# facebookresearch/pytorchvideo

Measured on AMD Instinct MI355X. Metric: clips/sec forward, higher is better.
Workload: dtype bf16; 1 GPU; x3d_m: create_x3d(input_clip_length=16,input_crop_size=224) [B,3,16,224,224]; per_gpu_batch=32, global_batch=32, parallelism=dp1 (batch-sharded, logits all_gather), head_collective=none (one rank: the logits stay where they are), hip_graph=True, streams=2

## Files before the change

### pytorchvideo_amd/accelerator/mi355x/emit.py

```python
import ctypes as C

import torch
import torch.nn as nn

from ... import _lib as L
from . import tuning
from .session import Ptr, pad8


class Unsupported(Exception):
    pass


def _cls_name(m):
    return getattr(m, "_orig_cls", type(m)).__name__


def _is_a(m, types):
    return issubclass(getattr(m, "_orig_cls", type(m)), types)


def act_code(act):
    if act is None or isinstance(act, nn.Identity):
        return L.ACT_NONE
# ... 484 lines not shown
        if getattr(se, "is_3d", True) is not True:
            raise Unsupported("2-D squeeze-excitation")
        _se_parts(se, x.C)
        y, psum, nblk = emit_dwconv(sess, conv_b, x, bn, L.ACT_NONE, want_psum=True, label="conv_b.dw+se")
        gate = emit_se_gate(sess, se, psum, nblk, x.B, x.C, y.voxels)
        sess.release(psum)
        return y, gate, act
    y = emit_conv(sess, conv_b, x, bn, act, label="conv_b")
    return y, None, L.ACT_NONE


def _conv_bc_desc(sess, bb, a, residual, out):
    conv_b, conv_c = bb.conv_b, bb.conv_c
    if not isinstance(conv_b, nn.Conv3d) or not isinstance(conv_c, nn.Conv3d) or sess.itemsize != 2 or a.f32:
        return None
    if conv_b.padding_mode != "zeros" or isinstance(conv_b.padding, str) or conv_c.padding_mode != "zeros" \
            or isinstance(conv_c.padding, str):
        return None
    bn, se = _split_norm_b(bb.norm_b)
    if se is not None or conv_b.groups != 1 or tuple(conv_b.dilation) != (1, 1, 1) or conv_b.in_channels != a.C:
        return None
    if conv_c.kernel_size != (1, 1, 1) or tuple(conv_c.stride) != (1, 1, 1) or _triple(conv_c.padding) != (0, 0, 0) \
            or conv_c.groups != 1 or conv_c.in_channels != conv_b.out_channels:
        return None
    if a.ld < pad8(a.C) or (residual is not None and residual.f32):
        return None
    kt, kh, kw = conv_b.kernel_size
    st, sh, sw = conv_b.stride
    pt, ph, pw = _triple(conv_b.padding)
    To, Ho, Wo = _conv_out(a.T, kt, st, pt), _conv_out(a.H, kh, sh, ph), _conv_out(a.W, kw, sw, pw)
    if min(To, Ho, Wo) <= 0 or kt * kh * kw == 1:
        return None
    cout2 = conv_c.out_channels
    if out is not None:
        if (out.B, out.T, out.H, out.W, out.C) != (a.B, To, Ho, Wo, cout2) or out.f32:
            return None
        ldy, y_bs = out.ld, out.bs
    else:
        ldy, y_bs = pad8(cout2), To * Ho * Wo * pad8(cout2)
    if residual is not None and ((residual.B, residual.T, residual.H, residual.W, residual.C) != (a.B, To, Ho, Wo, cout2)
                                 or residual.ld != ldy or residual.bs != y_bs):
        return None
    return dict(x_bs=a.bs, y_bs=y_bs, r_bs=y_bs if residual is not None else 0, ldx=a.ld, ldy=ldy,
                ldr=ldy if residual is not None else 0, B=a.B, Ti=a.T, Hi=a.H, Wi=a.W, cin=pad8(a.C), To=To, Ho=Ho, Wo=Wo,
                cout=conv_b.out_channels, kt=kt, kh=kh, kw=kw, st=st, sh=sh, sw=sw, pt=pt, ph=ph, pw=pw,
                dtype=sess.pv_dtype, pw2_cout=cout2)


def can_fuse_conv_bc(sess, bb, a, residual, out, shortcut):
    if not tuning.get("fuse_bc") or shortcut is not None:
        return False
    g = _conv_bc_desc(sess, bb, a, residual, out)
    if g is None:
        return False
    d = L.Conv3dDesc()
    for k, v in g.items():
        setattr(d, k, v)
    return L.lib().pv_conv3d_pw2_supported(C.byref(d)) == 1


def emit_fused_conv_bc(sess, bb, a, residual, final_act, out=None):
    g = _conv_bc_desc(sess, bb, a, residual, out)
    conv_b, conv_c = bb.conv_b, bb.conv_c
    bn, _ = _split_norm_b(bb.norm_b)
    cb, cc, cin_p = conv_b.out_channels, conv_c.out_channels, pad8(a.C)
    taps = g["kt"] * g["kh"] * g["kw"]
    y = out if out is not None else sess.alloc_act(a.B, g["To"], g["Ho"], g["Wo"], cc)
    wb = torch.zeros(cb, taps, cin_p, dtype=torch.float32)
    wb[:, :, : a.C] = conv_b.weight.detach().float().cpu().permute(0, 2, 3, 4, 1).reshape(cb, taps, a.C)
    wc = torch.zeros(cc, pad8(cb), dtype=torch.float32)
    wc[:, :cb] = conv_c.weight.detach().float().cpu().reshape(cc, cb)
    scale_b, shift_b = fold_norm(bn, cb, conv_b.bias)
    scale_c, shift_c = fold_norm(bb.norm_c, cc, conv_c.bias)
    aff_b = bn is not None and not isinstance(bn, nn.Identity)
    aff_c = bb.norm_c is not None and not isinstance(bb.norm_c, nn.Identity)
    f = dict(g)
    f.update(x=a.ptr, w=sess.add_weight(wb.to(sess.dtype)), y=y.ptr,
             scale=sess.add_weight(scale_b) if aff_b else None,
             shift=sess.add_weight(shift_b) if (aff_b or conv_b.bias is not None) else None,
             residual=residual.ptr if residual is not None else None,
             act=act_code(bb.act_b), a_act=L.ACT_NONE,
             pw2_w=sess.add_weight(wc.to(sess.dtype)),
             pw2_scale=sess.add_weight(scale_c) if aff_c else None,
             pw2_shift=sess.add_weight(shift_c) if (aff_c or conv_c.bias is not None) else None,
             pw2_act=final_act)
    vox_in, vox_out = a.B * a.voxels, y.B * y.voxels
    alg = sess.itemsize * (vox_in * cin_p + cb * taps * cin_p + cc * pad8(cb) + vox_out * pad8(cc)
                           + (vox_out * pad8(cc) if residual is not None else 0))
    flops = 2 * vox_out * (cb * taps * a.C + cc * cb)
    sess.add_op(L.OP_CONV3D, f, label="conv_bc|%dx%dx%dx%d c%d->%d->%d k%dx%dx%d s%d%d%d+k1x1x1" % (
        a.B, g["To"], g["Ho"], g["Wo"], a.C, cb, cc, g["kt"], g["kh"], g["kw"], g["st"], g["sh"], g["sw"]),
        alg_bytes=alg, flops=flops)
    return y


def emit_bottleneck(sess, bb, x, residual=None, final_act=L.ACT_NONE, out=None, shortcut=None):
    for name in ("conv_a", "conv_b", "conv_c"):
        if getattr(bb, name, None) is None:
            raise Unsupported("bottleneck without %s" % name)
    if can_fuse_bottleneck_ab(sess, bb, x):
        b, gate, deferred = emit_fused_conv_ab_se(sess, bb, x)
    elif can_fuse_pointwise_into_dw(sess, bb.conv_a, bb.conv_b, x):
        b, gate, deferred = emit_conv_b(sess, bb.conv_b, x, bb.norm_b, bb.act_b,
                                        producer=(bb.conv_a, bb.norm_a, act_code(bb.act_a)))
    else:
        a = emit_conv(sess, bb.conv_a, x, bb.norm_a, act_code(bb.act_a), label="conv_a")
        if can_fuse_conv_bc(sess, bb, a, residual, out, shortcut):
            c = emit_fused_conv_bc(sess, bb, a, residual, final_act, out=out)
            sess.release(a)
            return c
        b, gate, deferred = emit_conv_b(sess, bb.conv_b, a, bb.norm_b, bb.act_b)
        sess.release(a)
    check_conv3d(bb.conv_c)
    if (gate is not None or deferred != L.ACT_NONE) and \
            (bb.conv_c.kernel_size != (1, 1, 1) or bb.conv_c.stride != (1, 1, 1) or _triple(bb.conv_c.padding) != (0, 0, 0)):
        raise Unsupported("SE block whose conv_c is not pointwise")
    c = emit_conv(sess, bb.conv_c, b, bb.norm_c, final_act, residual=residual, a_gate=gate, a_act=deferred,
                  out=out, label="conv_c", shortcut=shortcut)
    sess.release(b)
    if gate is not None:
        sess.release(gate)
    return c


def pack_bottleneck_operands(conv_a, norm_a, conv_b, bn_b, conv_c, norm_c):
    cin, Cc = conv_a.in_channels, conv_a.out_channels
    cout = conv_c.out_channels if conv_c is not None else 16
    Cp, cin_p = (Cc + 31) // 32 * 32, (cin + 31) // 32 * 32

    def frag_image(w, rows_p, cols_p):
        wp = torch.zeros(rows_p, cols_p, dtype=torch.float32)
        wp[:w.shape[0], :w.shape[1]] = w
        return wp.reshape(rows_p // 16, 16, cols_p // 32, 4, 8).permute(0, 2, 3, 1, 4).contiguous().to(torch.bfloat16).reshape(-1)

    wa = frag_image(conv_a.weight.detach().float().cpu().reshape(Cc, cin), Cp, cin_p)
    wc = frag_image(conv_c.weight.detach().float().cpu().reshape(cout, Cc), (cout + 15) // 16 * 16, Cp) if conv_c is not None else None
    wb = torch.zeros(27, Cp, dtype=torch.float32)
    wb[:, :Cc] = conv_b.weight.detach().float().cpu().reshape(Cc, 27).t()

    def padded(v, n):
        o = torch.zeros(n, dtype=torch.float32)
        o[:v.numel()] = v
        return o

    sa, ha = fold_norm(norm_a, Cc, conv_a.bias)
    sb, hb = fold_norm(bn_b, Cc, conv_b.bias)
    out = dict(wa=wa, wb=wb.reshape(-1), sa=padded(sa, Cp), ha=padded(ha, Cp), sb=padded(sb, Cp), hb=padded(hb, Cp))
    if conv_c is not None:
        sc, hc = fold_norm(norm_c, cout, conv_c.bias)
        out.update(wc=wc, sc=sc, hc=hc)
    return out


def _bottleneck_geometry_ok(sess, bb, x, want_se):
    if not tuning.get("fuse_block") or sess.itemsize != 2 or x.f32:
        return None
    ca, cb, cc = getattr(bb, "conv_a", None), getattr(bb, "conv_b", None), getattr(bb, "conv_c", None)
    if not all(isinstance(c, nn.Conv3d) for c in (ca, cb, cc)):
        return None
    try:
        bn_b, se = _split_norm_b(bb.norm_b)
        if (se is not None) != want_se or check_conv3d(ca) or not check_conv3d(cb) or check_conv3d(cc) or group_width(cb) != 1:
            return None
        if se is not None:
            if getattr(se, "is_3d", True) is not True:
                return None
            _se_parts(se, cb.out_channels)
        acts = (act_code(bb.act_a), act_code(bb.act_b))
    except Unsupported:
        return None
    for c in (ca, cc):
        if c.kernel_size != (1, 1, 1) or c.stride != (1, 1, 1) or _triple(c.padding) != (0, 0, 0) or c.groups != 1:
            return None
    if cb.kernel_size != (3, 3, 3) or cb.stride != (1, 1, 1) or _triple(cb.padding) != (1, 1, 1) or _triple(cb.dilation) != (1, 1, 1):
        return None
    if ca.in_channels != x.C or ca.out_channels != cb.in_channels or cb.out_channels != cc.in_channels:
        return None
    if x.bs != x.voxels * x.ld:
        return None
    return acts


def can_fuse_bottleneck(sess, bb, x, residual, final_act=L.ACT_RELU):
    if residual is not x:
        return False
    acts = _bottleneck_geometry_ok(sess, bb, x, want_se=False)
    if acts is None or bb.conv_c.out_channels != x.C:
        return False
    d = L.BottleneckDesc()
    d.B, d.T, d.H, d.W, d.cin, d.C, d.cout = x.B, x.T, x.H, x.W, x.C, bb.conv_a.out_channels, bb.conv_c.out_channels
    d.ldx, d.ldy, d.ldr, d.dtype, d.mode = x.ld, pad8(bb.conv_c.out_channels), x.ld, sess.pv_dtype, L.BLOCK_FULL
    d.act_a, d.act_b, d.act_out = acts[0], acts[1], final_act
    return L.lib().pv_bottleneck_supported(C.byref(d)) == 1


def can_fuse_bottleneck_ab(sess, bb, x):
    acts = _bottleneck_geometry_ok(sess, bb, x, want_se=True)
    if acts is None:
        return False
    d = L.BottleneckDesc()
    d.B, d.T, d.H, d.W, d.cin, d.C, d.cout = x.B, x.T, x.H, x.W, x.C, bb.conv_a.out_channels, bb.conv_c.out_channels
    d.ldx, d.ldy, d.dtype, d.mode, d.act_a = x.ld, pad8(bb.conv_a.out_channels), sess.pv_dtype, L.BLOCK_AB, acts[0]
    return L.lib().pv_bottleneck_supported(C.byref(d)) == 1


def emit_fused_conv_ab_se(sess, bb, x):
    bn_b, se = _split_norm_b(bb.norm_b)
    ops = pack_bottleneck_operands(bb.conv_a, bb.norm_a, bb.conv_b, bn_b, None, None)
    cin, Cc = bb.conv_a.in_channels, bb.conv_a.out_channels
    y = sess.alloc_act(x.B, x.T, x.H, x.W, Cc)
    f = dict(x=x.ptr, y=y.ptr, residual=None, wc=None, sc=None, hc=None, x_bs=x.bs, y_bs=y.bs, r_bs=0, ldx=x.ld, ldy=y.ld, ldr=0,
             B=x.B, T=x.T, H=x.H, W=x.W, cin=cin, C=Cc, cout=bb.conv_c.out_channels,
             act_a=act_code(bb.act_a), act_b=L.ACT_NONE, act_out=L.ACT_NONE, dtype=sess.pv_dtype, mode=L.BLOCK_AB)
    for k in ("wa", "wb", "sa", "ha", "sb", "hb"):
        f[k] = sess.add_weight(ops[k])
    d = L.BottleneckDesc()
    d.H, d.W, d.cin, d.C, d.cout, d.ldx, d.mode, d.dtype = x.H, x.W, cin, Cc, bb.conv_c.out_channels, x.ld, L.BLOCK_AB, sess.pv_dtype
    nblk = L.lib().pv_bottleneck_psum_blocks(C.byref(d))
    if nblk <= 0:
        raise Unsupported("bottleneck geometry")
    psum = sess.alloc_raw(4 * x.B * nblk * pad8(Cc))
    f["psum"] = psum
    vox = x.B * x.T * x.H * x.W
    sess.add_op(L.OP_BOTTLENECK, f, label="conv_ab.fused+se|%dx%dx%dx%d c%d->%d k1x1x1+k3x3x3 psum" % (x.B, x.T, x.H, x.W, cin, Cc),
                alg_bytes=sess.itemsize * vox * (pad8(cin) + pad8(Cc)) + 2 * Cc * cin + 108 * Cc, flops=2 * vox * Cc * (cin + 27))
    gate = emit_se_gate(sess, se, psum, nblk, x.B, Cc, x.T * x.H * x.W)
    sess.release(psum)
    return y, gate, act_code(bb.act_b)


def emit_fused_bottleneck(sess, bb, x, final_act, out=None):
    bn_b, _ = _split_norm_b(bb.norm_b)
    ops = pack_bottleneck_operands(bb.conv_a, bb.norm_a, bb.conv_b, bn_b, bb.conv_c, bb.norm_c)
    cin, Cc, cout = bb.conv_a.in_channels, bb.conv_a.out_channels, bb.conv_c.out_channels
    y = out if out is not None else sess.alloc_act(x.B, x.T, x.H, x.W, cout)
    f = dict(x=x.ptr, y=y.ptr, residual=x.ptr, x_bs=x.bs, y_bs=y.bs, r_bs=x.bs, ldx=x.ld, ldy=y.ld, ldr=x.ld,
             B=x.B, T=x.T, H=x.H, W=x.W, cin=cin, C=Cc, cout=cout,
             act_a=act_code(bb.act_a), act_b=act_code(bb.act_b), act_out=final_act, dtype=sess.pv_dtype, mode=L.BLOCK_FULL, psum=None)
    for k in ("wa", "wb", "wc", "sa", "ha", "sb", "hb", "sc", "hc"):
        f[k] = sess.add_weight(ops[k])
    vox = x.B * x.T * x.H * x.W
    sess.add_op(L.OP_BOTTLENECK, f, label="block.fused|%dx%dx%dx%d c%d->%d->%d k1x1x1+k3x3x3+k1x1x1" % (x.B, x.T, x.H, x.W, cin, Cc, cout),
                alg_bytes=sess.itemsize * vox * (pad8(cin) + pad8(cout)) + 2 * Cc * (cin + cout) + 108 * Cc,
                flops=2 * vox * Cc * (cin + cout + 27))
    return y


def emit_res_block(sess, rb, x, out=None):
    if not is_add_fusion(rb.branch_fusion):
        raise Unsupported("branch_fusion is not a sum")
    if _cls_name(rb.branch2) != "BottleneckBlock":
        raise Unsupported("branch2 is %s" % _cls_name(rb.branch2))
    bb = rb.branch2
    if rb.branch1_conv is not None and isinstance(getattr(bb, "conv_c", None), nn.Conv3d) \
            and can_fold_shortcut(sess, bb.conv_c, rb.branch1_conv, x, bb.conv_c.in_channels):
        return emit_bottleneck(sess, bb, x, residual=None, final_act=act_code(rb.activation), out=out,
                               shortcut=(rb.branch1_conv, rb.branch1_norm, x))
    if rb.branch1_conv is None and can_fuse_bottleneck(sess, bb, x, x, act_code(rb.activation)):
        return emit_fused_bottleneck(sess, bb, x, act_code(rb.activation), out=out)
    if rb.branch1_conv is None:
        shortcut = x
    else:
        shortcut = emit_conv(sess, rb.branch1_conv, x, rb.branch1_norm, L.ACT_NONE, label="shortcut")
    y = emit_bottleneck(sess, rb.branch2, x, residual=shortcut, final_act=act_code(rb.activation), out=out)
    if shortcut is not x:
        sess.release(shortcut)
    return y


def emit_res_stage(sess, stage, x, out=None):
    cur = x
    n = len(stage.res_blocks)
    for i, blk in enumerate(stage.res_blocks):
        if _cls_name(blk) != "ResBlock":
            raise Unsupported("stage element %s" % _cls_name(blk))
        nxt = emit_res_block(sess, blk, cur, out=out if i == n - 1 else None)
        if cur is not x:
            sess.release(cur)
        cur = nxt
    return cur


def can_fuse_temporal_dw(sess, first, second, mid_norm, mid_act, x, act):
    if not tuning.get("fuse_stem") or x.ld != 4 or sess.itemsize != 2:
        return False
    if mid_norm is not None and not isinstance(mid_norm, nn.Identity):
        return False
    if mid_act != L.ACT_NONE or not isinstance(first, nn.Conv3d) or not isinstance(second, nn.Conv3d):
        return False
    try:
        if check_conv3d(first) or not check_conv3d(second):
            return False
    except Unsupported:
        return False
    if group_width(second) != 1:
        return False
    k = second.kernel_size
    if first.bias is not None or first.out_channels != second.in_channels or second.in_channels != second.out_channels:
        return False
    if k[1:] != (1, 1) or second.stride != (1, 1, 1) or _triple(second.padding) != (k[0] // 2, 0, 0) or k[0] % 2 == 0:
        return False
    kt, kh, kw = first.kernel_size
    st, sh, sw = first.stride
    pt, ph, pw = _triple(first.padding)
    d = L.Conv3dDesc()
    d.ldx, d.cin, d.cout, d.dtype, d.act, d.dwt_k = 4, 4, first.out_channels, sess.pv_dtype, act, k[0]
    d.B, d.Ti, d.Hi, d.Wi = x.B, x.T, x.H, x.W
    d.To, d.Ho, d.Wo = _conv_out(x.T, kt, st, pt), _conv_out(x.H, kh, sh, ph), _conv_out(x.W, kw, sw, pw)
    d.kt, d.kh, d.kw, d.st, d.sh, d.sw, d.pt, d.ph, d.pw = kt, kh, kw, st, sh, sw, pt, ph, pw
    return min(d.To, d.Ho, d.Wo) > 0 and L.lib().pv_conv3d_dwt_supported(C.byref(d)) == 1


def emit_stem(sess, stem, x, out=None):
    act = act_code(stem.activation)
    conv = stem.conv
    if _cls_name(conv) == "Conv2plus1d":
        first, second = (conv.conv_xy, conv.conv_t) if conv.conv_xy_first else (conv.conv_t, conv.conv_xy)
        if can_fuse_temporal_dw(sess, first, second, conv.norm, act_code(conv.activation), x, act):
            y = emit_conv(sess, first, x, stem.norm, act, out=out if stem.pool is None else None,
                          label="stem.conv01", dwt=second)
        else:
            mid = emit_conv(sess, first, x, conv.norm, act_code(conv.activation), label="stem.conv0")
            y = emit_conv(sess, second, mid, stem.norm, act, out=out if stem.pool is None else None,
                          label="stem.conv1")
            sess.release(mid)
    else:
        y = emit_conv(sess, conv, x, stem.norm, act, out=out if stem.pool is None else None, label="stem.conv")
    if stem.pool is not None:
        p = emit_pool(sess, stem.pool, y, out=out, label="stem.pool")
        sess.release(y)
        y = p
    return y


def _emit_linear_rows(sess, lin, x, act=L.ACT_NONE, y_f32=False, label="linear"):
    if not isinstance(lin, nn.Linear):
        raise Unsupported("%s is not nn.Linear" % _cls_name(lin))
    if lin.in_features != x.C:
        raise RuntimeError("Linear expects %d features, got %d" % (lin.in_features, x.C))
    conv = nn.Conv3d(lin.in_features, lin.out_features, 1, bias=lin.bias is not None)
    conv.weight.data = lin.weight.detach().reshape(lin.out_features, lin.in_features, 1, 1, 1)
    if lin.bias is not None:
        conv.bias.data = lin.bias.detach()
    return emit_conv(sess, conv, x, None, act, y_f32=y_f32, label=label)


def emit_projected_pool(sess, pp, x):
    a = emit_conv(sess, pp.pre_conv, x, pp.pre_norm, act_code(pp.pre_act), label="head.pre_conv")
    p = emit_pool(sess, pp.pool, a, label="head.pool")
    sess.release(a)
    y = emit_conv(sess, pp.post_conv, p, pp.post_norm, act_code(pp.post_act), label="head.post_conv")
    sess.release(p)
    return y


def emit_res_head(sess, head, x):
    cur = x
    if head.pool is not None:
        if _cls_name(head.pool) == "ProjectedPool":
            cur = emit_projected_pool(sess, head.pool, x)
        else:
            cur = emit_pool(sess, head.pool, x, label="head.pool")
    if head.dropout is not None and not isinstance(head.dropout, nn.Dropout):
        raise Unsupported("head dropout %s" % _cls_name(head.dropout))
    a = head.activation
    if a is not None and not isinstance(a, (nn.Softmax, nn.Sigmoid, nn.ReLU)):
        raise Unsupported("head activation %s" % _cls_name(a))
    act = L.ACT_SIGMOID if isinstance(a, nn.Sigmoid) else (L.ACT_RELU if isinstance(a, nn.ReLU) else L.ACT_NONE)
    logits = _emit_linear_rows(sess, head.proj, cur, act=act, y_f32=True, label="head.proj")
    if cur is not x:
        sess.release(cur)
    if isinstance(a, nn.Softmax):
        if a.dim != 1:
            raise Unsupported("softmax over dim %s" % a.dim)
        f = dict(x=logits.ptr, y=logits.ptr, gamma=None, beta=None, rows=logits.B * logits.voxels, C=logits.C,
                 ldx=logits.ld, ldy=logits.ld, rows_per_batch=0, eps=0.0, dtype=L.PV_F32)
        sess.add_op(L.OP_SOFTMAX_ROWS, f, label="head.softmax")
    if head.output_pool is None:
        return logits
# ... 228 lines not shown
```

### pytorchvideo_amd/accelerator/mi355x/tuning.py

```python

OPTIONS = {
    "fuse_shortcut": True,
    "stem_wpair": True,
    "fuse_ab": True,
    "fuse_ab_max_cin": 64,
    "fuse_block": True,
    "fuse_bc": True,
    "fuse_stem": True,
    "stem_ncdhw": True,
    "fuse_kv_pool": True,
    "fuse_posenc": True,
    "split_joint_graph": True,
    "pool_stream_min_elems": 1 << 22,
    "fuse_ln_qkv": True,
    "fuse_ln_qkv_max_c": 192,
    "fuse_next_norm": True,
    "fuse_mlp": True,
    "arena_margin": 0,
    "arena_guards": 0,
}


def get(name):
    return OPTIONS[name]


def apply(spec):
    from ... import _lib as L
    for item in [t for t in (spec or "").split(",") if t]:
        k, v = item.split("=")
        if k in OPTIONS:
            OPTIONS[k] = type(OPTIONS[k])(int(v))
        else:
            L.tune(**{k: int(v)})
```

### pytorchvideo_amd/csrc/pv_block.hip

```cpp
#include "pv_common.h"

namespace {

constexpr int kTH = 2;
constexpr int kHR = kTH + 2;
constexpr int kWP = 16;
constexpr int kTW = 14;

template <int CP, int KSA, int COUTP, bool PAIR, int SEGS> struct BlkGeom {
  static constexpr int NI = PAIR ? CP / 2 : CP;
  static constexpr int WPR = (NI + 63) / 64;
  static constexpr int NWS = kTW / SEGS;
  static constexpr int SWAVES = kTH * SEGS * WPR;
  static constexpr int MWAVES = kHR * kWP / 16;
  static constexpr int MTA = CP / 16;
  static constexpr int KSC = CP / 32;
  static constexpr int MTC = COUTP / 16;
  static constexpr int TPW = (MTC * kTH + MWAVES - 1) / MWAVES;
  static constexpr int E_STRIDE = CP * 2 + 8;
  static constexpr int MID_STRIDE = CP * 2 + 16;
  static constexpr int OUT_STRIDE = COUTP * 2 + 8;
  static constexpr int WA_BYTES = MTA * KSA * 1024;
  static constexpr int E_BYTES = kHR * kWP * E_STRIDE;
  static constexpr int MID_BYTES = kTH * kWP * MID_STRIDE;
// ... 183 lines not shown
            const float v3 = c4[k][3] * s4[3] + h4[3] + __uint_as_float(res[k][1] & 0xffff0000u);
            unsigned o0 = pack2(v0, v1), o1 = pack2(v2, v3);
            if (out_relu) { o0 = relu2(o0); o1 = relu2(o1); }
            *reinterpret_cast<u32x2*>(ob + k * 64) = u32x2{o0, o1};
          }
        }
      }
      if constexpr (ABL != 4) __syncthreads();
      if constexpr (ABL == 8) __syncthreads();
    }
  } else {
    const int sw = wave - G::MWAVES;
    const int wpart = sw % G::WPR, rs = sw / G::WPR;
    const int seg = rs % SEGS, srow = rs / SEGS;
    const int item = wpart * 64 + lane;
    constexpr int IB = PAIR ? 4 : 2;
    constexpr int IC = PAIR ? 2 : 1;
    const bool p_ok = item < G::NI;
    const unsigned psel = (item & 1) ? 0x03020c0cu : 0x01000c0cu;
    const int pch = p_ok ? IC * item : 0;
    vt wt[27];
#pragma unroll
    for (int t = 0; t < 27; ++t) wt[t] = V::ldw(d.wb + (long)t * CP + pch, p_ok);
    const vt sb2 = V::ldw(d.sb + pch, p_ok), hb2 = V::ldw(d.hb + pch, p_ok);
    vt acc[3][G::NWS];
#pragma unroll
    for (int a = 0; a < 3; ++a)
#pragma unroll
      for (int n = 0; n < G::NWS; ++n) acc[a][n] = V::zero();
    const int soh = h0 + srow, sow0 = w0 + seg * G::NWS;
    const bool st_ok = MODE == 1 && p_ok && pch < pv_round_up(d.C, 8) && soh < H;
    bf16_t* Mp = static_cast<bf16_t*>(d.y) + (long)b * d.y_bs;
    const unsigned yplane_b = (unsigned)(H * W * d.ldy) * 2u, yvox_b = (unsigned)d.ldy * 2u;
    __amdgpu_buffer_rsrc_t ryo = __builtin_amdgcn_make_buffer_rsrc((void*)Mp, 0, (int)(yplane_b * (unsigned)T), 0x00020000);
    const unsigned m_off = (unsigned)((soh * W + sow0) * d.ldy + pch) * 2u;
    vt ps = V::zero();
    constexpr int CH = COUTP * 2 / 16;
    constexpr int ITEMS = kTH * kWP * CH, ROUNDS = (ITEMS + 255) / 256;
    unsigned o_src[ROUNDS], o_dst[ROUNDS];
#pragma unroll
    for (int r = 0; r < ROUNDS; ++r) {
      const int it = r * 256 + sw * 64 + lane;
      const int slot = it / CH, chunk = it - slot * CH;
      const int orow = slot / kWP, ocol = slot - orow * kWP;
      const bool ok = MODE == 0 && it < ITEMS && h0 + orow < H && ocol < kTW && w0 + ocol < W && chunk * 8 < cout_p8;
      o_src[r] = (unsigned)((it < ITEMS ? slot : 0) * G::OUT_STRIDE + chunk * 16);
      o_dst[r] = ok ? (unsigned)(((h0 + orow) * W + w0 + ocol) * d.ldy) * 2u + (unsigned)chunk * 16u : 0x80000000u;
    }

    for (int i = 0; i <= T + 3; ++i) {
      if (MODE == 0 && i >= 4 && ABL != 3) {
        const unsigned char* ob = s_out + ((i - 4) & 1) * G::OUT_BYTES;
        const unsigned tb = (unsigned)(i - 4) * yplane_b;
#pragma unroll
        for (int r = 0; r < ROUNDS; ++r) {
          const u32x2 lo = *reinterpret_cast<const u32x2*>(ob + o_src[r]);
          const u32x2 hi = *reinterpret_cast<const u32x2*>(ob + o_src[r] + 8);
          const u32x4 v = {lo[0], lo[1], hi[0], hi[1]};
          __builtin_amdgcn_raw_buffer_store_b128(v, ryo, (int)(o_dst[r] + tb), 0, 0);
        }
      }
      const int p = i - 1;
      if (p_ok && p >= 0 && p <= T) {
        if (p < T) {
          const unsigned char* ebase = s_e + (p & 1) * G::E_BYTES + (seg * G::NWS) * G::E_STRIDE + (PAIR ? item : item >> 1) * 4;
#pragma unroll
          for (int dh = 0; dh < 3; ++dh) {
            vt xv[G::NWS + 2];
            if constexpr (ABL == 9) {
#pragma unroll
              for (int c = G::NWS + 1; c >= 0; --c) { xv[c] = V::load(ebase + ((srow + dh) * kWP + c) * G::E_STRIDE, psel); asm volatile("" : "+v"(xv[c])); }
            } else {
#pragma unroll
              for (int c = 0; c < G::NWS + 2; ++c) {
                xv[c] = V::load(ebase + ((srow + dh) * kWP + c) * G::E_STRIDE, psel);
                if constexpr (ABL == 11) asm volatile("" : "+v"(xv[c]));
              }
              if constexpr (ABL == 12) __builtin_amdgcn_s_waitcnt(0xc07f);
            }
#pragma unroll
            for (int dw = 0; dw < 3; ++dw) {
              const vt w0v = wt[(0 * 3 + dh) * 3 + dw];
              const vt w1v = wt[(1 * 3 + dh) * 3 + dw];
              const vt w2v = wt[(2 * 3 + dh) * 3 + dw];
#pragma unroll
              for (int n = 0; n < G::NWS; ++n) {
                if constexpr (ABL != 1) {
                  V::fma(acc[2][n], xv[n + dw], w0v);
                  V::fma(acc[1][n], xv[n + dw], w1v);
                  V::fma(acc[0][n], xv[n + dw], w2v);
                } else {
                  asm volatile("" :: "v"(xv[n + dw]));
                }
              }
            }
          }
        }
        if (p >= 1) {
          if constexpr (MODE == 0) {
            unsigned char* mbase = s_mid + ((p - 1) & 1) * G::MID_BYTES + (srow * kWP + seg * G::NWS) * G::MID_STRIDE + item * IB;
#pragma unroll
            for (int n = 0; n < G::NWS; ++n) {
              if constexpr (PAIR) {
                float v0 = acc[0][n].x * sb2.x + hb2.x, v1 = acc[0][n].y * sb2.y + hb2.y;
                if (ACT_B == PV_ACT_RELU) { v0 = fmaxf(v0, 0.f); v1 = fmaxf(v1, 0.f); }
                else if (ACT_B == PV_ACT_SWISH && ABL != 6) { v0 *= pv_sigmoid(v0); v1 *= pv_sigmoid(v1); }
                *reinterpret_cast<unsigned*>(mbase + n * G::MID_STRIDE) = pack2(v0, v1);
              } else {
                float v0 = acc[0][n] * sb2 + hb2;
                if (ACT_B == PV_ACT_RELU) v0 = fmaxf(v0, 0.f);
                else if (ACT_B == PV_ACT_SWISH && ABL != 6) v0 *= pv_sigmoid(v0);
                *reinterpret_cast<bf16_t*>(mbase + n * G::MID_STRIDE) = (bf16_t)v0;
                if constexpr (ABL == 13) __builtin_amdgcn_sched_barrier(0);
              }
            }
          } else {
            const unsigned tb = (unsigned)(p - 1) * yplane_b;
#pragma unroll
            for (int n = 0; n < G::NWS; ++n) {
              const bool ok = st_ok && sow0 + n < W;
              const unsigned off = (ok ? m_off + (unsigned)n * yvox_b : 0x80000000u) + tb;
              if constexpr (PAIR) {
                const float v0 = acc[0][n].x * sb2.x + hb2.x, v1 = acc[0][n].y * sb2.y + hb2.y;
                if (ok) { ps.x += v0; ps.y += v1; }
                __builtin_amdgcn_raw_buffer_store_b32(pack2(v0, v1), ryo, (int)off, 0, 0);
              } else {
                const float v0 = acc[0][n] * sb2 + hb2;
                if (ok) ps += v0;
                __builtin_amdgcn_raw_buffer_store_b16(__builtin_bit_cast(unsigned short, (bf16_t)v0), ryo, (int)off, 0, 0);
              }
            }
          }
        }
#pragma unroll
        for (int n = 0; n < G::NWS; ++n) {
          acc[0][n] = acc[1][n];
          acc[1][n] = acc[2][n];
          acc[2][n] = V::zero();
        }
      }
      if constexpr (ABL != 4) __syncthreads();
      if constexpr (ABL == 8) __syncthreads();
    }
    if (MODE == 1 && d.psum != nullptr && p_ok && pch < pv_round_up(d.C, 8)) {
      const int c_p = pv_round_up(d.C, 8);
      const long blk = ((long)(tile_h * kTH + srow) * tiles_w + tile_w) * SEGS + seg;
      float* dst = d.psum + ((long)b * ((long)tiles_h * kTH * tiles_w * SEGS) + blk) * c_p + pch;
      if constexpr (PAIR) *reinterpret_cast<float2*>(dst) = soh < H ? ps : float2{0.f, 0.f};
      else *dst = soh < H ? ps : 0.f;
    }
  }
}

int check(const pv_bottleneck_desc& d) {
  if (d.mode != PV_BLOCK_FULL && d.mode != PV_BLOCK_AB) return PV_ERR_INVALID;
  if (!d.x || !d.y || !d.wa || !d.wb || !d.sa || !d.ha || !d.sb || !d.hb) return PV_ERR_INVALID;
  if (d.B <= 0 || d.T <= 0 || d.H <= 0 || d.W <= 0 || d.cin <= 0 || d.C <= 0 || d.cout <= 0) return PV_ERR_INVALID;
  if (d.ldx < pv_round_up(d.cin, 8) || d.ldx % 8) return PV_ERR_INVALID;
  if (d.mode == PV_BLOCK_FULL) {
    if (!d.wc || !d.sc || !d.hc) return PV_ERR_INVALID;
    if (d.ldy < pv_round_up(d.cout, 8) || d.ldy % 8) return PV_ERR_INVALID;
    if (d.residual && (d.ldr < pv_round_up(d.cout, 8) || d.ldr % 4)) return PV_ERR_INVALID;
  } else if (d.ldy < pv_round_up(d.C, 8) || d.ldy % 2) {
    return PV_ERR_INVALID;
  }
  return PV_OK;
}

int variant_of(const pv_bottleneck_desc& d) {
  const int cp = pv_round_up(d.C, 32), cinp = pv_round_up(d.cin, 32);
  const bool c_out = d.mode != PV_BLOCK_AB;
  if (cp == 224 && cinp == 96 && d.ldx >= 96 && (!c_out || d.cout == 96)) return 4;
  if (cp == 128 && cinp == 64 && (!c_out || d.cout == 48)) return 3;
  if (cp == 64 && cinp == 32 && (!c_out || d.cout == 24)) return 2;
  return 0;
}

template <int CP, int KSA, int COUTP, bool PAIR, int SEGS>
int launch_variant(const pv_bottleneck_desc& d, dim3 grid, int tiles_h, int tiles_w, hipStream_t s) {
  const dim3 block(512);
  if (d.mode == PV_BLOCK_AB) PV_LAUNCH((bottleneck_block_kernel<CP, KSA, COUTP, PAIR, SEGS, PV_ACT_NONE, 1>), grid, block, 0, s, d, tiles_h, tiles_w);
  else if (d.act_b == PV_ACT_SWISH) PV_LAUNCH((bottleneck_block_kernel<CP, KSA, COUTP, PAIR, SEGS, PV_ACT_SWISH, 0>), grid, block, 0, s, d, tiles_h, tiles_w);
  else if (d.act_b == PV_ACT_RELU) PV_LAUNCH((bottleneck_block_kernel<CP, KSA, COUTP, PAIR, SEGS, PV_ACT_RELU, 0>), grid, block, 0, s, d, tiles_h, tiles_w);
  else PV_LAUNCH((bottleneck_block_kernel<CP, KSA, COUTP, PAIR, SEGS, PV_ACT_NONE, 0>), grid, block, 0, s, d, tiles_h, tiles_w);
  PV_LAUNCH_CHECK();
  return PV_OK;
}

}

extern "C" int pv_bottleneck_supported(const pv_bottleneck_desc* dp) {
  if (!dp) return 0;
  const pv_bottleneck_desc& d = *dp;
  if (d.dtype != PV_BF16) return 0;
  if (d.B <= 0 || d.T <= 0 || d.H <= 0 || d.W <= 0) return 0;
  if (d.mode != PV_BLOCK_FULL && d.mode != PV_BLOCK_AB) return 0;
  if (d.act_a != PV_ACT_RELU && d.act_a != PV_ACT_NONE) return 0;
  if (d.mode == PV_BLOCK_FULL) {
    if (d.act_b != PV_ACT_SWISH && d.act_b != PV_ACT_RELU && d.act_b != PV_ACT_NONE) return 0;
    if (d.act_out != PV_ACT_RELU && d.act_out != PV_ACT_NONE) return 0;
  }
  if ((long)d.T * d.H * d.W * (d.ldx > d.ldy ? d.ldx : d.ldy) * 2 > 0x7fffffffL) return 0;
  if ((long)d.B * pv_ceil_div(d.H, kTH) * pv_ceil_div(d.W, kTW) > 0x7fffffffL) return 0;
  const int v = variant_of(d);
  if (!v) return 0;
  const int stages = d.mode == PV_BLOCK_FULL ? pv_tune("block_stages", 0x1c) : pv_tune("block_stages_ab", 0x10);
  return (stages >> v) & 1;
}

extern "C" int pv_bottleneck_psum_blocks(const pv_bottleneck_desc* dp) {
  if (!dp) return 0;
  const int segs = variant_of(*dp) == 4 ? 1 : 2;
  return (int)(pv_ceil_div(dp->H, kTH) * kTH * pv_ceil_div(dp->W, kTW) * segs);
}

extern "C" int pv_bottleneck(const pv_bottleneck_desc* dp, pv_stream_t stream) {
  if (!dp) return PV_ERR_INVALID;
  const int rc = check(*dp);
  if (rc != PV_OK) return rc;
  if (!pv_bottleneck_supported(dp)) return PV_ERR_UNSUPPORTED;
  const pv_bottleneck_desc& d = *dp;
  hipStream_t s = static_cast<hipStream_t>(stream);
  const int tiles_h = (int)pv_ceil_div(d.H, kTH), tiles_w = (int)pv_ceil_div(d.W, kTW);
  const dim3 grid((unsigned)(d.B * tiles_h * tiles_w));
#ifdef PV_DEV_ABLATION
  if (const int abl = pv_tune("block_abl", 0); abl && abl < 8 && variant_of(d) == 4 && d.mode == PV_BLOCK_FULL && d.act_b == PV_ACT_SWISH) {
    const dim3 block(512);
    switch (abl) {
      case 1: PV_LAUNCH((bottleneck_block_kernel<224, 3, 96, true, 1, PV_ACT_SWISH, 0, 1>), grid, block, 0, s, d, tiles_h, tiles_w); break;
      case 2: PV_LAUNCH((bottleneck_block_kernel<224, 3, 96, true, 1, PV_ACT_SWISH, 0, 2>), grid, block, 0, s, d, tiles_h, tiles_w); break;
      case 3: PV_LAUNCH((bottleneck_block_kernel<224, 3, 96, true, 1, PV_ACT_SWISH, 0, 3>), grid, block, 0, s, d, tiles_h, tiles_w); break;
      case 4: PV_LAUNCH((bottleneck_block_kernel<224, 3, 96, true, 1, PV_ACT_SWISH, 0, 4>), grid, block, 0, s, d, tiles_h, tiles_w); break;
      default: PV_LAUNCH((bottleneck_block_kernel<224, 3, 96, true, 1, PV_ACT_SWISH, 0, 6>), grid, block, 0, s, d, tiles_h, tiles_w); break;
    }
    PV_LAUNCH_CHECK();
    return PV_OK;
  }
#endif
#ifdef PV_DEV_ABLATION
  if (const int abl = pv_tune("block_abl", 0); abl >= 8 && variant_of(d) == 2 && d.mode == PV_BLOCK_FULL && d.act_b == PV_ACT_SWISH) {
    const dim3 block(512);
    switch (abl) {
      case 8: PV_LAUNCH((bottleneck_block_kernel<64, 1, 32, false, 2, PV_ACT_SWISH, 0, 8>), grid, block, 0, s, d, tiles_h, tiles_w); break;
      case 9: PV_LAUNCH((bottleneck_block_kernel<64, 1, 32, false, 2, PV_ACT_SWISH, 0, 9>), grid, block, 0, s, d, tiles_h, tiles_w); break;
      case 11: PV_LAUNCH((bottleneck_block_kernel<64, 1, 32, false, 2, PV_ACT_SWISH, 0, 11>), grid, block, 0, s, d, tiles_h, tiles_w); break;
      case 12: PV_LAUNCH((bottleneck_block_kernel<64, 1, 32, false, 2, PV_ACT_SWISH, 0, 12>), grid, block, 0, s, d, tiles_h, tiles_w); break;
      case 13: PV_LAUNCH((bottleneck_block_kernel<64, 1, 32, false, 2, PV_ACT_SWISH, 0, 13>), grid, block, 0, s, d, tiles_h, tiles_w); break;
      default: PV_LAUNCH((bottleneck_block_kernel<64, 1, 32, true, 2, PV_ACT_SWISH, 0, 0>), grid, block, 0, s, d, tiles_h, tiles_w); break;
    }
    PV_LAUNCH_CHECK();
    return PV_OK;
  }
#endif
  switch (variant_of(d)) {
    case 4: return launch_variant<224, 3, 96, true, 1>(d, grid, tiles_h, tiles_w, s);
    case 3: return launch_variant<128, 2, 48, true, 2>(d, grid, tiles_h, tiles_w, s);
    case 2: return launch_variant<64, 1, 32, false, 2>(d, grid, tiles_h, tiles_w, s);
  }
  return PV_ERR_UNSUPPORTED;
}
```

Before: 11200 clips/s.

## Add plane-tiled fused conv_a+conv_b kernel for 448-channel 7x7 stage, including strided entry

Adds a new fused bottleneck kernel for the last X3D stage (448 mid channels, 7x7 output). Some waves compute the 1x1x1 conv_a with MFMA into a double-buffered LDS plane, while others run the depthwise 3x3x3 conv_b over time with a rolling accumulator. It also covers the stride-(1,2,2) first block and blocks without SE. This removes the intermediate conv_a activation round-trip through HBM and some launches. The cost is a large LDS footprint and a grid sized by channel slices and time segments, which may give low occupancy.

```diff
diff --git a/pytorchvideo_amd/accelerator/mi355x/emit.py b/pytorchvideo_amd/accelerator/mi355x/emit.py
--- a/pytorchvideo_amd/accelerator/mi355x/emit.py
+++ b/pytorchvideo_amd/accelerator/mi355x/emit.py
@@ -660,7 +660,7 @@
     return out
 
 
-def _bottleneck_geometry_ok(sess, bb, x, want_se):
+def _bottleneck_geometry_ok(sess, bb, x, want_se, strides=((1, 1, 1),)):
     if not tuning.get("fuse_block") or sess.itemsize != 2 or x.f32:
         return None
     ca, cb, cc = getattr(bb, "conv_a", None), getattr(bb, "conv_b", None), getattr(bb, "conv_c", None)
@@ -680,7 +680,7 @@
     for c in (ca, cc):
         if c.kernel_size != (1, 1, 1) or c.stride != (1, 1, 1) or _triple(c.padding) != (0, 0, 0) or c.groups != 1:
             return None
-    if cb.kernel_size != (3, 3, 3) or cb.stride != (1, 1, 1) or _triple(cb.padding) != (1, 1, 1) or _triple(cb.dilation) != (1, 1, 1):
+    if cb.kernel_size != (3, 3, 3) or tuple(cb.stride) not in strides or _triple(cb.padding) != (1, 1, 1) or _triple(cb.dilation) != (1, 1, 1):
         return None
     if ca.in_channels != x.C or ca.out_channels != cb.in_channels or cb.out_channels != cc.in_channels:
         return None
@@ -702,13 +702,33 @@
     return L.lib().pv_bottleneck_supported(C.byref(d)) == 1
 
 
+def _plane_widths(cin, Cc):
+    plane = (Cc + 31) // 32 * 32 == 448
+    return plane, plane and (cin + 31) // 32 * 32 == 96
+
+
 def can_fuse_bottleneck_ab(sess, bb, x):
-    acts = _bottleneck_geometry_ok(sess, bb, x, want_se=True)
+    try:
+        se = _split_norm_b(getattr(bb, "norm_b", None))[1] is not None
+    except Unsupported:
+        return False
+    acts = _bottleneck_geometry_ok(sess, bb, x, want_se=se, strides=((1, 1, 1), (1, 2, 2)))
     if acts is None:
         return False
+    cin, Cc = x.C, bb.conv_a.out_channels
+    plane, strided = _plane_widths(cin, Cc)
+    if plane and not tuning.get("fuse_plane"):
+        return False
+    if (tuple(bb.conv_b.stride) != (1, 1, 1)) != strided or (not se and not plane):
+        return False
+    if plane:
+        out_hw = ((x.H - 1) // 2 + 1, (x.W - 1) // 2 + 1) if strided else (x.H, x.W)
+        if out_hw != (7, 7):
+            return False
     d = L.BottleneckDesc()
-    d.B, d.T, d.H, d.W, d.cin, d.C, d.cout = x.B, x.T, x.H, x.W, x.C, bb.conv_a.out_channels, bb.conv_c.out_channels
-    d.ldx, d.ldy, d.dtype, d.mode, d.act_a = x.ld, pad8(bb.conv_a.out_channels), sess.pv_dtype, L.BLOCK_AB, acts[0]
+    d.B, d.T, d.H, d.W, d.cin, d.C, d.cout = x.B, x.T, x.H, x.W, cin, Cc, bb.conv_c.out_channels
+    d.ldx, d.ldy, d.dtype, d.mode, d.act_a = x.ld, pad8(Cc), sess.pv_dtype, L.BLOCK_AB, acts[0]
+    d.act_b = L.ACT_NONE if se else acts[1]
     return L.lib().pv_bottleneck_supported(C.byref(d)) == 1
 
 
@@ -716,23 +736,32 @@
     bn_b, se = _split_norm_b(bb.norm_b)
     ops = pack_bottleneck_operands(bb.conv_a, bb.norm_a, bb.conv_b, bn_b, None, None)
     cin, Cc = bb.conv_a.in_channels, bb.conv_a.out_channels
-    y = sess.alloc_act(x.B, x.T, x.H, x.W, Cc)
+    strided = tuple(bb.conv_b.stride) != (1, 1, 1)
+    Ho, Wo = ((x.H - 1) // 2 + 1, (x.W - 1) // 2 + 1) if strided else (x.H, x.W)
+    act_b = L.ACT_NONE if se is not None else act_code(bb.act_b)
+    y = sess.alloc_act(x.B, x.T, Ho, Wo, Cc)
     f = dict(x=x.ptr, y=y.ptr, residual=None, wc=None, sc=None, hc=None, x_bs=x.bs, y_bs=y.bs, r_bs=0, ldx=x.ld, ldy=y.ld, ldr=0,
              B=x.B, T=x.T, H=x.H, W=x.W, cin=cin, C=Cc, cout=bb.conv_c.out_channels,
-             act_a=act_code(bb.act_a), act_b=L.ACT_NONE, act_out=L.ACT_NONE, dtype=sess.pv_dtype, mode=L.BLOCK_AB)
+             act_a=act_code(bb.act_a), act_b=act_b, act_out=L.ACT_NONE, dtype=sess.pv_dtype, mode=L.BLOCK_AB, psum=None)
     for k in ("wa", "wb", "sa", "ha", "sb", "hb"):
         f[k] = sess.add_weight(ops[k])
+    vox_in, vox = x.B * x.T * x.H * x.W, x.B * x.T * Ho * Wo
+    alg_bytes = sess.itemsize * (vox_in * pad8(cin) + vox * pad8(Cc)) + 2 * Cc * cin + 108 * Cc
+    flops = 2 * Cc * (vox_in * cin + vox * 27)
+    geom = "%dx%dx%dx%d c%d->%d k1x1x1+k3x3x3%s" % (x.B, x.T, Ho, Wo, cin, Cc, " s122" if strided else "")
+    if se is None:
+        sess.add_op(L.OP_BOTTLENECK, f, label="conv_ab.fused|" + geom, alg_bytes=alg_bytes, flops=flops)
+        return y, None, L.ACT_NONE
     d = L.BottleneckDesc()
-    d.H, d.W, d.cin, d.C, d.cout, d.ldx, d.mode, d.dtype = x.H, x.W, cin, Cc, bb.conv_c.out_channels, x.ld, L.BLOCK_AB, sess.pv_dtype
+    d.B, d.T, d.H, d.W, d.cin, d.C, d.cout = x.B, x.T, x.H, x.W, cin, Cc, bb.conv_c.out_channels
+    d.ldx, d.mode, d.dtype = x.ld, L.BLOCK_AB, sess.pv_dtype
     nblk = L.lib().pv_bottleneck_psum_blocks(C.byref(d))
     if nblk <= 0:
         raise Unsupported("bottleneck geometry")
     psum = sess.alloc_raw(4 * x.B * nblk * pad8(Cc))
     f["psum"] = psum
-    vox = x.B * x.T * x.H * x.W
-    sess.add_op(L.OP_BOTTLENECK, f, label="conv_ab.fused+se|%dx%dx%dx%d c%d->%d k1x1x1+k3x3x3 psum" % (x.B, x.T, x.H, x.W, cin, Cc),
-                alg_bytes=sess.itemsize * vox * (pad8(cin) + pad8(Cc)) + 2 * Cc * cin + 108 * Cc, flops=2 * vox * Cc * (cin + 27))
-    gate = emit_se_gate(sess, se, psum, nblk, x.B, Cc, x.T * x.H * x.W)
+    sess.add_op(L.OP_BOTTLENECK, f, label="conv_ab.fused+se|" + geom + " psum", alg_bytes=alg_bytes, flops=flops)
+    gate = emit_se_gate(sess, se, psum, nblk, x.B, Cc, x.T * Ho * Wo)
     sess.release(psum)
     return y, gate, act_code(bb.act_b)
 
diff --git a/pytorchvideo_amd/accelerator/mi355x/tuning.py b/pytorchvideo_amd/accelerator/mi355x/tuning.py
--- a/pytorchvideo_amd/accelerator/mi355x/tuning.py
+++ b/pytorchvideo_amd/accelerator/mi355x/tuning.py
@@ -5,6 +5,7 @@
     "fuse_ab": True,
     "fuse_ab_max_cin": 64,
     "fuse_block": True,
+    "fuse_plane": True,
     "fuse_bc": True,
     "fuse_stem": True,
     "stem_ncdhw": True,
diff --git a/pytorchvideo_amd/csrc/pv_block.hip b/pytorchvideo_amd/csrc/pv_block.hip
--- a/pytorchvideo_amd/csrc/pv_block.hip
+++ b/pytorchvideo_amd/csrc/pv_block.hip
@@ -359,6 +359,226 @@
   }
 }
 
+constexpr int kPSL = 72;
+constexpr int kPMT = 5;
+constexpr int kPEC = kPMT * 16;
+constexpr int kPNSL = 6;
+constexpr int kPO = 7;
+constexpr int kPSW = 4;
+
+template <int S, int KSA, int MW> struct PlaneGeom {
+  static constexpr int PW = S * (kPO - 1) + 3;
+  static constexpr int NTILES = (S * kPO * S * kPO + 15) / 16;
+  static constexpr int NT = (NTILES + MW - 1) / MW;
+  static constexpr int NX = S * (kPO - 1) + 3;
+  static constexpr int E_STRIDE = kPEC * 2 + 8;
+  static constexpr int E_BYTES = PW * PW * E_STRIDE;
+  static constexpr int WA_BYTES = kPMT * KSA * 1024;
+  static constexpr int TOTAL = WA_BYTES + 2 * E_BYTES + 2 * kPEC * 4;
+  static_assert(E_BYTES % 8 == 0 && TOTAL <= 160 * 1024, "LDS");
+};
+
+template <int S, int KSA, int MW>
+__global__ __launch_bounds__((MW + kPSW) * 64, S == 1 ? 3 : 2) void bottleneck_plane_kernel(const pv_bottleneck_desc d, int nseg, int Ho, int Wo) {
+  using G = PlaneGeom<S, KSA, MW>;
+  constexpr int NTHR = (MW + kPSW) * 64;
+  using V = SV<true>;
+  __shared__ __attribute__((aligned(16))) unsigned char smem[G::TOTAL];
+  unsigned char* const s_wa = smem;
+  unsigned char* const s_e = s_wa + G::WA_BYTES;
+  float* const s_sa = reinterpret_cast<float*>(s_e + 2 * G::E_BYTES);
+  float* const s_ha = s_sa + kPEC;
+
+  const int tid = threadIdx.x;
+  const int lane = tid & 63;
+  const int wave = __builtin_amdgcn_readfirstlane(tid >> 6);
+  const int n16 = lane & 15, q = lane >> 4;
+  const int b = blockIdx.x % d.B;
+  const int rest = blockIdx.x / d.B;
+  const int slice = rest % kPNSL, seg = rest / kPNSL;
+  const int T = d.T, H = d.H, W = d.W;
+  const int t0 = seg * T / nseg, t1 = (seg + 1) * T / nseg;
+  const int pa = t0 > 0 ? t0 - 1 : 0, pb = t1 < T ? t1 : T - 1;
+  const int iters = t1 - pa + 2;
+  const int c0 = slice * kPSL, mt0 = c0 >> 4, coff = c0 & 15;
+
+  {
+    const u32x4* wa = static_cast<const u32x4*>(d.wa) + (long)mt0 * KSA * 64;
+    u32x4* la = reinterpret_cast<u32x4*>(s_wa);
+    for (int i = tid; i < G::WA_BYTES / 16; i += NTHR) la[i] = wa[i];
+    u32x2* le = reinterpret_cast<u32x2*>(s_e);
+    for (int i = tid; i < 2 * G::E_BYTES / 8; i += NTHR) le[i] = u32x2{0u, 0u};
+    for (int i = tid; i < kPEC; i += NTHR) { s_sa[i] = d.sa[mt0 * 16 + i]; s_ha[i] = d.ha[mt0 * 16 + i]; }
+  }
+  __syncthreads();
+
+  if (wave < MW) {
+    constexpr unsigned kOOB = 0x80000000u;
+    const bf16_t* X = static_cast<const bf16_t*>(d.x) + (long)b * d.x_bs;
+    const unsigned plane_b = (unsigned)(H * W * d.ldx) * 2u;
+    __amdgpu_buffer_rsrc_t rx = __builtin_amdgcn_make_buffer_rsrc((void*)X, 0, (int)(plane_b * (unsigned)T), 0x00020000);
+    unsigned x_off[G::NT];
+    int e_dst[G::NT];
+    bool vox_ok[G::NT];
+#pragma unroll
+    for (int k = 0; k < G::NT; ++k) {
+      const int v = (wave + MW * k) * 16 + n16;
+      vox_ok[k] = v < H * W;
+      const int hh = v / W, ww = v - hh * W;
+      x_off[k] = vox_ok[k] ? (unsigned)(v * d.ldx + q * 8) * 2u : kOOB;
+      e_dst[k] = ((hh + 1) * G::PW + ww + 1) * G::E_STRIDE + q * 8;
+    }
+    const bool a_relu = d.act_a == PV_ACT_RELU;
+    u32x4 xf[G::NT][KSA];
+    auto load_x = [&](int k, int p) {
+#pragma unroll
+      for (int ks = 0; ks < KSA; ++ks)
+        xf[k][ks] = __builtin_amdgcn_raw_buffer_load_b128(rx, (int)(x_off[k] + (unsigned)p * plane_b + (unsigned)ks * 64u), 0, 0);
+    };
+#pragma unroll
+    for (int k = 0; k < G::NT; ++k) load_x(k, pa);
+    for (int i = 0; i < iters; ++i) {
+      if (pa + i <= pb) {
+        unsigned char* const eb = s_e + (i & 1) * G::E_BYTES;
+#pragma unroll
+        for (int k = 0; k < G::NT; ++k) {
+          if ((wave + MW * k) * 16 < H * W) {
+            f32x4 c4[kPMT];
+#pragma unroll
+            for (int mt = 0; mt < kPMT; ++mt) c4[mt] = f32x4{0.f, 0.f, 0.f, 0.f};
+#pragma unroll
+            for (int ks = 0; ks < KSA; ++ks)
+#pragma unroll
+              for (int mt = 0; mt < kPMT; ++mt) {
+                const bf16x8 af = *reinterpret_cast<const bf16x8*>(s_wa + ((mt * KSA + ks) * 64 + lane) * 16);
+                c4[mt] = __builtin_amdgcn_mfma_f32_16x16x32_bf16(af, __builtin_bit_cast(bf16x8, xf[k][ks]), c4[mt], 0, 0, 0);
+              }
+            if (pa + i < pb) load_x(k, pa + i + 1);
+#pragma unroll
+            for (int mt = 0; mt < kPMT; ++mt) {
+              const f32x4 s4 = *reinterpret_cast<const f32x4*>(s_sa + mt * 16 + q * 4);
+              const f32x4 h4 = *reinterpret_cast<const f32x4*>(s_ha + mt * 16 + q * 4);
+              unsigned o0 = pack2(c4[mt][0] * s4[0] + h4[0], c4[mt][1] * s4[1] + h4[1]);
+              unsigned o1 = pack2(c4[mt][2] * s4[2] + h4[2], c4[mt][3] * s4[3] + h4[3]);
+              if (a_relu) { o0 = relu2(o0); o1 = relu2(o1); }
+              if (vox_ok[k]) *reinterpret_cast<u32x2*>(eb + e_dst[k] + mt * 32) = u32x2{o0, o1};
+            }
+          }
+        }
+      }
+      __syncthreads();
+    }
+  } else {
+    typedef V::T vt;
+    const int item = (wave - MW) * 64 + lane;
+    const int row = item / (kPSL / 2), pair = item - row * (kPSL / 2);
+    const bool r_ok = row < Ho;
+    const int pch = c0 + 2 * pair;
+    const int c_p8 = pv_round_up(d.C, 8), c_p32 = pv_round_up(d.C, 32);
+    const bool st_ok = r_ok && pch < c_p8;
+    vt wt[27];
+#pragma unroll
+    for (int t = 0; t < 27; ++t) wt[t] = V::ldw(d.wb + (long)t * c_p32 + pch, r_ok);
+    const vt sb2 = V::ldw(d.sb + pch, r_ok), hb2 = V::ldw(d.hb + pch, r_ok);
+    vt acc[3][kPO];
+#pragma unroll
+    for (int a = 0; a < 3; ++a)
+#pragma unroll
+      for (int n = 0; n < kPO; ++n) acc[a][n] = V::zero();
+    bf16_t* Yp = static_cast<bf16_t*>(d.y) + (long)b * d.y_bs;
+    const unsigned yplane_b = (unsigned)(Ho * Wo * d.ldy) * 2u, yvox_b = (unsigned)d.ldy * 2u;
+    __amdgpu_buffer_rsrc_t ryo = __builtin_amdgcn_make_buffer_rsrc((void*)Yp, 0, (int)(yplane_b * (unsigned)T), 0x00020000);
+    const unsigned y_off = (unsigned)(row * Wo * d.ldy + pch) * 2u;
+    const int act_b = d.act_b;
+    vt ps = V::zero();
+    const unsigned char* const ebase = s_e + (r_ok ? S * row * G::PW : 0) * G::E_STRIDE + coff * 2 + pair * 4;
+
+    for (int i = 0; i < iters; ++i) {
+      const int p = pa + i - 1;
+      if (r_ok && i >= 1) {
+        if (p < T) {
+          const unsigned char* ep = ebase + ((i - 1) & 1) * G::E_BYTES;
+          unsigned raw[G::NX];
+#pragma unroll
+          for (int c = 0; c < G::NX; ++c) raw[c] = *reinterpret_cast<const unsigned*>(ep + c * G::E_STRIDE);
+#pragma unroll
+          for (int dh = 0; dh < 3; ++dh) {
+            vt xv[G::NX];
+#pragma unroll
+            for (int c = 0; c < G::NX; ++c) xv[c] = float2{__uint_as_float(raw[c] << 16), __uint_as_float(raw[c] & 0xffff0000u)};
+            if (dh < 2) {
+#pragma unroll
+              for (int c = 0; c < G::NX; ++c) raw[c] = *reinterpret_cast<const unsigned*>(ep + ((dh + 1) * G::PW + c) * G::E_STRIDE);
+            }
+#pragma unroll
+            for (int dw = 0; dw < 3; ++dw) {
+              const vt w0v = wt[(0 * 3 + dh) * 3 + dw];
+              const vt w1v = wt[(1 * 3 + dh) * 3 + dw];
+              const vt w2v = wt[(2 * 3 + dh) * 3 + dw];
+#pragma unroll
+              for (int n = 0; n < kPO; ++n) {
+                V::fma(acc[2][n], xv[S * n + dw], w0v);
+                V::fma(acc[1][n], xv[S * n + dw], w1v);
+                V::fma(acc[0][n], xv[S * n + dw], w2v);
+              }
+            }
+            if (dh < 2) {
+#pragma unroll
+              for (int c = 0; c < G::NX; ++c) {
+                const int n = c * kPO / G::NX;
+                asm volatile("" : "+v"(raw[c]) : "v"(acc[0][n].x), "v"(acc[1][n].x), "v"(acc[2][n].x));
+              }
+            }
+          }
+        }
+        if (p - 1 >= t0) {
+          const unsigned tb = (unsigned)(p - 1) * yplane_b;
+#pragma unroll
+          for (int n = 0; n < kPO; ++n) {
+            const bool ok = st_ok && n < Wo;
+            const unsigned off = (ok ? y_off + (unsigned)n * yvox_b : 0x80000000u) + tb;
+            float v0 = acc[0][n].x * sb2.x + hb2.x, v1 = acc[0][n].y * sb2.y + hb2.y;
+            if (ok) { ps.x += v0; ps.y += v1; }
+            if (act_b == PV_ACT_SWISH) { v0 *= pv_sigmoid(v0); v1 *= pv_sigmoid(v1); }
+            else if (act_b == PV_ACT_RELU) { v0 = fmaxf(v0, 0.f); v1 = fmaxf(v1, 0.f); }
+            __builtin_amdgcn_raw_buffer_store_b32(pack2(v0, v1), ryo, (int)off, 0, 0);
+          }
+        }
+#pragma unroll
+        for (int n = 0; n < kPO; ++n) {
+          acc[0][n] = acc[1][n];
+          acc[1][n] = acc[2][n];
+          acc[2][n] = V::zero();
+        }
+      }
+      __syncthreads();
+    }
+    if (d.psum != nullptr && st_ok) {
+      float* dst = d.psum + ((long)b * ((long)nseg * Ho) + (long)seg * Ho + row) * c_p8 + pch;
+      *reinterpret_cast<float2*>(dst) = ps;
+    }
+  }
+}
+
+int plane_form(const pv_bottleneck_desc& d) {
+  if (d.mode != PV_BLOCK_AB || pv_round_up(d.C, 32) != 448 || d.C > kPSL * kPNSL) return 0;
+  const int cinp = pv_round_up(d.cin, 32);
+  if (d.ldx < cinp) return 0;
+  if (cinp == 192 && d.H <= kPO && d.W <= kPO) return 1;
+  if (cinp == 96 && d.H <= 2 * kPO && d.W <= 2 * kPO) return 2;
+  return 0;
+}
+int plane_out(int form, int n) { return form == 2 ? (n - 1) / 2 + 1 : n; }
+
+int plane_segments(const pv_bottleneck_desc& d, int form) {
+  int want = pv_tune("block_plane_tseg", 0);
+  if (want <= 0) want = (form == 1 ? 512 : 256) / (d.B * kPNSL);
+  if (want < 1) want = 1;
+  if (want > d.T) want = d.T;
+  const int len = (int)pv_ceil_div(d.T, want);
+  return (int)pv_ceil_div(d.T, len);
+}
+
 int check(const pv_bottleneck_desc& d) {
   if (d.mode != PV_BLOCK_FULL && d.mode != PV_BLOCK_AB) return PV_ERR_INVALID;
   if (!d.x || !d.y || !d.wa || !d.wb || !d.sa || !d.ha || !d.sb || !d.hb) return PV_ERR_INVALID;
@@ -403,20 +623,25 @@
   if (d.B <= 0 || d.T <= 0 || d.H <= 0 || d.W <= 0) return 0;
   if (d.mode != PV_BLOCK_FULL && d.mode != PV_BLOCK_AB) return 0;
   if (d.act_a != PV_ACT_RELU && d.act_a != PV_ACT_NONE) return 0;
-  if (d.mode == PV_BLOCK_FULL) {
-    if (d.act_b != PV_ACT_SWISH && d.act_b != PV_ACT_RELU && d.act_b != PV_ACT_NONE) return 0;
-    if (d.act_out != PV_ACT_RELU && d.act_out != PV_ACT_NONE) return 0;
-  }
+  if (d.act_b != PV_ACT_SWISH && d.act_b != PV_ACT_RELU && d.act_b != PV_ACT_NONE) return 0;
+  if (d.mode == PV_BLOCK_FULL && d.act_out != PV_ACT_RELU && d.act_out != PV_ACT_NONE) return 0;
   if ((long)d.T * d.H * d.W * (d.ldx > d.ldy ? d.ldx : d.ldy) * 2 > 0x7fffffffL) return 0;
   if ((long)d.B * pv_ceil_div(d.H, kTH) * pv_ceil_div(d.W, kTW) > 0x7fffffffL) return 0;
+  if (const int form = plane_form(d)) {
+    if ((long)d.B * kPNSL * plane_segments(d, form) > 0x7fffffffL) return 0;
+    return pv_tune("block_plane", 1) ? 1 : 0;
+  }
   const int v = variant_of(d);
   if (!v) return 0;
+  if (d.mode == PV_BLOCK_AB && d.act_b != PV_ACT_NONE) return 0;
   const int stages = d.mode == PV_BLOCK_FULL ? pv_tune("block_stages", 0x1c) : pv_tune("block_stages_ab", 0x10);
   return (stages >> v) & 1;
 }
 
 extern "C" int pv_bottleneck_psum_blocks(const pv_bottleneck_desc* dp) {
   if (!dp) return 0;
+  if (const int form = plane_form(*dp))
+    return dp->B > 0 && dp->T > 0 ? plane_segments(*dp, form) * plane_out(form, dp->H) : 0;
   const int segs = variant_of(*dp) == 4 ? 1 : 2;
   return (int)(pv_ceil_div(dp->H, kTH) * kTH * pv_ceil_div(dp->W, kTW) * segs);
 }
@@ -428,6 +653,14 @@
   if (!pv_bottleneck_supported(dp)) return PV_ERR_UNSUPPORTED;
   const pv_bottleneck_desc& d = *dp;
   hipStream_t s = static_cast<hipStream_t>(stream);
+  if (const int form = plane_form(d)) {
+    const int nseg = plane_segments(d, form), Ho = plane_out(form, d.H), Wo = plane_out(form, d.W);
+    const dim3 pgrid((unsigned)(d.B * kPNSL * nseg));
+    if (form == 1) PV_LAUNCH((bottleneck_plane_kernel<1, 6, 2>), pgrid, dim3(384), 0, s, d, nseg, Ho, Wo);
+    else PV_LAUNCH((bottleneck_plane_kernel<2, 3, 4>), pgrid, dim3(512), 0, s, d, nseg, Ho, Wo);
+    PV_LAUNCH_CHECK();
+    return PV_OK;
+  }
   const int tiles_h = (int)pv_ceil_div(d.H, kTH), tiles_w = (int)pv_ceil_div(d.W, kTW);
   const dim3 grid((unsigned)(d.B * tiles_h * tiles_w));
 #ifdef PV_DEV_ABLATION
```

New measurement: 11050 clips/s. 0.987x the previous value.
